# facebookresearch/momentum

Measured on AMD Instinct MI355X. Metric: character IK solves/sec (72-joint, 10 GN iters), higher is better.
Workload: dtype f32; 1 GPU; BASELINE configs[1]: B x 72-joint humanoid, P=128, pos+ori on 16 landmarks (M=192), GN lambda=0.05, 10 it; batch_per_gpu=4096, global_batch=4096, joints=72, params=128, rows=192, solved_parameters=96, route=fused, line_search=0, precision=f32

## Files before the change

momentum_amd/csrc/mmx_fused.hip:

```cpp
#include "mmx_device.hpp"
#include "mmx_fused_helpers.hpp"
#include "mmx_kernels.hpp"
#include "mmx_mixed.hpp"
#include "mmx_tree.hpp"

#include <cfloat>
#include <cstdlib>

namespace mmx {

struct MixRowRec {
  int4 q{0, 0, 0, 0};
  bool has = false;
};
template <typename Gather, typename Store>
__device__ __forceinline__ void mixTransformRows(const RigView& rig, int tid, Gather x, Store out, const MixRowRec& regRec = MixRowRec{}) {
  if (regRec.has) {
    if (tid < rig.numRowRec) {
      const int4 q = regRec.q;
      const int row = q.x & 0xffff, span = int(uint32_t(q.x) >> 16), in0 = q.y & 0xffff, cnt = int(uint32_t(q.y) >> 16);
      auto acc = __int_as_float(q.z) * x(in0);
      for (int k = q.w + 1; k < q.w + cnt; ++k) {
        acc += rig.ptValue[k] * x(rig.ptInner[k]);
      }
// ... 195 lines not shown
  }
  __syncthreads();
  for (int r = 0; r < rig.jumpRounds; ++r) {
    int next = -1;
    if (target >= 0) {
      const double* t = m.Y + kTanD * target;
#pragma unroll
      for (int c = 0; c < 7; ++c) {
        acc[c] += t[c];
      }
      next = reinterpret_cast<const int*>(t + 7)[0];
    }
    __syncthreads();
    if (target >= 0) {
      double* o = m.Y + kTanD * tid;
#pragma unroll
      for (int c = 0; c < 7; ++c) {
        o[c] = acc[c];
      }
      reinterpret_cast<int*>(o + 7)[0] = next;
    }
    target = next;
    __syncthreads();
  }
}

template <class FV>
__device__ __forceinline__ void mixApply(
    const RigView& rig, const FV& fd, const FusedLds& s, const MixLds& m, const int16_t* parentPos, int J, int NP, int n, int nsrc, double mu, const double* p, double* q, int tid, const MixRowRec& regRec = MixRowRec{}) {
  mixTangent(
      rig, fd, m, parentPos, J, tid,
      [&](int c) {
        const int cs = fd.colToSolve[c];
        return cs >= 0 ? p[cs] : 0.0;
      },
      regRec);
  mixAdjoint(
      fd, s, m, J, NP, n, nsrc, tid,
      [&](int u, int k, const D3& pu) {
        const double* pre = m.Y + kTanD * k;
        D3 v = dcross(D3{pre[3], pre[4], pre[5]}, pu);
        if (u < fd.Kp) {
          v = D3{pre[0], pre[1], pre[2]} + v + (kLn2D * pre[6]) * pu;
        }
        const double sg = m.us[u];
        return (sg * sg) * v;
      },
      q);
  for (int c = tid; c < n; c += 256) {
    q[c] += mu * p[c];
  }
  __syncthreads();
}

constexpr int kGenEv = 29;

template <int NB, bool kTR, bool kGen, int kRule>
struct FusedFour {
  static constexpr bool value = NB <= 6 && !kGen && !kTR;
};

struct FusedLayout {
  size_t uyFloats;
  size_t auxOff;
  size_t cellOff;
  size_t t9;
  size_t arenaFloats;
  size_t umomFloats;
  size_t regionFloats;
  size_t genFloats;
  size_t total;
};
__host__ __device__ inline FusedLayout fusedLayout(int NB, int J, int P, int U, int nsrc, int n, int numCells, bool cellsBehindRho, int GT, int genRows, bool separateUy = false, size_t csrFloats = 0, bool mix = false) {
  auto a4 = [](size_t x) { return (x + 3) & ~size_t(3); };
  auto h4 = [&](size_t x) { return a4((x + 1) / 2); };
  auto mx = [](size_t x, size_t y) { return x > y ? x : y; };
  const size_t T = size_t(NB) * (NB + 1) / 2, NP = 16 * size_t(NB);
  FusedLayout l;
  l.cellOff = cellsBehindRho ? 2 * NP : 0;
  const size_t aux = a4(mx(2 * NP, mx(size_t(nsrc), l.cellOff + size_t(numCells))));
  l.auxOff = separateUy ? a4(3 * size_t(U)) : 0;
  l.uyFloats = separateUy ? l.auxOff + aux : mx(a4(3 * size_t(U)), aux);
  l.t9 = a4(size_t(kTan) * J);
  l.arenaFloats = mx(size_t(kSrcCh - 1) * size_t(srcStrideFor(nsrc)), 2 * l.t9 + a4(P));
  if (mix) {
    l.arenaFloats = mx(size_t(kSrcCh - 1) * size_t(srcStrideFor(nsrc)), a4(2 * (mixXDoubles(J, nsrc) + mixYDoubles(J, P))));
  }
  l.umomFloats = mx(a4(size_t(kUmom) * U), a4(size_t(kC1) * J));
  const size_t scratch = fkBufFloats(J) + 2 * a4(size_t(kC2) * J) + l.umomFloats;
  l.regionFloats = mx(scratch, T * 256);
  const size_t rowsGp = a4(size_t(genRows));
  l.genFloats = GT > 0 ? a4(size_t(kGenEv) * GT) + 2 * a4(rowsGp) + a4(rowsGp * size_t(srcStrideFor(int(NP)))) : 0;
  const size_t meta = h4(NP + 1) + 3 * a4(nsrc) + a4(J) + 4 * h4(J) + h4(size_t(J) + 1) + 2 * h4(U) + h4(n) + h4(P);
  size_t fixed = a4(P) + a4(size_t(kJs) * J) + 2 * a4(3 * size_t(U)) + a4(U) + 2 * a4(NP) + l.uyFloats + 16 + 8;
  if (mix) {
    fixed = l.uyFloats + 40 + 8 + a4(2 * mixPersistentDoubles(J, P, U, int(NP))) + 2 * h4(J);
  }
  l.total = meta + fixed + l.genFloats + l.arenaFloats + l.regionFloats + csrFloats;
  return l;
}

__device__ __forceinline__ double generalRowsError(const ProblemDev& pb, const float* js, int b, int tid) {
  double e = 0.0;
  for (int g = tid; g < pb.G; g += 256) {
    const JointBlockDev k = jointBlockOf(pb, b, pb.genBlock[g]);
    e += double(evalJointConstraint(k, js, pb.genJoint[g], jointBlockSecondJoint(pb, k, g), size_t(b) * size_t(k.count) + size_t(g - k.first)).werr);
  }
  if (pb.wLimit > 0.f) {
    const float tWeightE = 1e+1f * pb.wLimit;
    for (int q = tid; q < pb.NE; q += 256) {
      e += double(evalEllipsoid(pb.ellipsoids[q], js, tWeightE).werr);
    }
  }
  return e;
}

__device__ __forceinline__ double generalRowsEvaluate(const ProblemDev& pb, const float* js, int b, int U, int tid, float* gEv, float* gRes) {
  double e = 0.0;
  int* evi = reinterpret_cast<int*>(gEv);
  for (int g = tid; g < pb.G; g += 256) {
    const JointBlockDev k = jointBlockOf(pb, b, pb.genBlock[g]);
    const int i = g - k.first;
    const JointEval o = evalJointConstraint(k, js, pb.genJoint[g], jointBlockSecondJoint(pb, k, g), size_t(b) * size_t(k.count) + size_t(i));
    const int row = k.rowStart + o.nrows * i - 3 * U;
    e += double(o.werr);
    for (int q = 0; q < o.nrows; ++q) {
      gRes[row + q] = o.sigma * o.f[q];
    }
    const float sg = fabsf(o.sigma) <= 1e-9f ? 0.f : o.sigma;
    float* w = gEv + kGenEv * g;
    w[0] = o.vp.x, w[1] = o.vp.y, w[2] = o.vp.z;
    w[3] = o.vn.x, w[4] = o.vn.y, w[5] = o.vn.z;
#pragma unroll
    for (int q = 0; q < 9; ++q) {
      w[6 + q] = sg * o.dp[q];
      w[15 + q] = sg * o.dn[q];
    }
    evi[kGenEv * g + 24] = pb.genTin[g];
    evi[kGenEv * g + 25] = row;
    evi[kGenEv * g + 26] = jointEvalFlags(o);
    evi[kGenEv * g + 27] = jointBlockSecondTin(pb, k, g);
  }
  const float tWeightE = 1e+1f * pb.wLimit;
  for (int q = tid; q < pb.NE; q += 256) {
    const EllipsoidDev ct = pb.ellipsoids[q];
    const int row = pb.rowsJoint - 3 * pb.NE + 3 * q - 3 * U, g = pb.G + q;
    EllipsoidEval o = evalEllipsoid(ct, js, tWeightE);
    if (!(pb.wLimit > 0.f)) {
      o.jwgt = o.werr = 0.f;
    }
    e += double(o.werr);
    gRes[row] = o.diff.x * o.jwgt, gRes[row + 1] = o.diff.y * o.jwgt, gRes[row + 2] = o.diff.z * o.jwgt;
    float* w = gEv + kGenEv * g;
    w[0] = o.position.x, w[1] = o.position.y, w[2] = o.position.z;
    w[3] = w[4] = w[5] = 0.f;
#pragma unroll
    for (int k = 0; k < 9; ++k) {
      w[6 + k] = (k == 0 || k == 4 || k == 8) ? o.jwgt : 0.f;
      w[15 + k] = 0.f;
    }
    evi[kGenEv * g + 24] = ct.tinParent;
    evi[kGenEv * g + 25] = row;
    evi[kGenEv * g + 26] = 3 | 16;
    evi[kGenEv * g + 27] = ct.tinStop;
  }
  return e;
}

struct GenSlot {
// ... 505 lines not shown
  SolveStateDev st;
  FusedParams fp;
};
static __global__ void stashFusedArgsKernel(FusedArgs a, FusedArgs* dst) {
  *dst = a;
}
template <int NB, int MODE, bool kTR, bool kGen = false, int kRule = -1, bool kArgLazy = false, bool kMix = false>
__global__ void __launch_bounds__(256, (NB <= 6 && !kGen ? (FusedFour<NB, kTR, kGen, kRule>::value && !kMix ? 4 : 3) : (NB <= 8 ? 2 : 1))) fusedSolveKernel(
    const FusedArgs* __restrict__ argsDev,
    const RigDev rigArg,
    const ProblemDev pbArg,
    FusedDev fdV,
    float* __restrict__ theta,
    SolveStateDev stV,
    FusedParams fpV,
    float* __restrict__ dbgH,
    float* __restrict__ dbgG,
    long long* __restrict__ dbgClk,
    MixSelect sel) {
  static_assert(!kMix || (!kTR && !kGen && kRule == -1 && !kArgLazy), "the mixed-precision instantiation: generic rule, reference rows");
  constexpr int T = NB * (NB + 1) / 2;
  constexpr int NP = 16 * NB;
  constexpr bool kLook = NB <= 8;
  long long clkLast = 0;
  const int dbgStop = (MODE == 2 && dbgClk != nullptr) ? int(dbgClk[31]) : 0;
#define MMX_CLK(slot)                                             \
  if (MODE == 2 && blockIdx.x == 0 && threadIdx.x == 0) {         \
    const long long now_ = clock64();                             \
    dbgClk[slot] += now_ - clkLast;                               \
    clkLast = now_;                                               \
  }                                                               \
  if (MODE == 2 && dbgStop == (slot) + 1) {                       \
    __builtin_amdgcn_endpgm();                                    \
  }
  extern __shared__ __attribute__((aligned(16))) float smem[];
  int bSel = blockIdx.x;
  if (kMix && sel.map != nullptr) {
    if (int(blockIdx.x) >= *sel.count) {
      return;
    }
    bSel = sel.map[blockIdx.x];
  }
  const int b = bSel, tid = threadIdx.x;
  const int wave = tid >> 6, lane = tid & 63;
  RigDev rigV;
  ProblemDev pbV;
  if (!kArgLazy) {
    rigV = rigArg;
    pbV = pbArg;
    selectInstanceRig(rigV, b);
    selectInstanceWeights(pbV, b);
  }
  const RigDev& rig = kArgLazy ? argsDev->rig : rigV;
  const ProblemDev& pb = kArgLazy ? argsDev->pb : pbV;
  const FusedDev& fd = kArgLazy ? argsDev->fd : fdV;
  const SolveStateDev& st = kArgLazy ? argsDev->st : stV;
  const FusedParams& fp = kArgLazy ? argsDev->fp : fpV;
  const int J = rig.J, P = rig.P, U = fd.U, n = fd.n, nsrc = fd.nsrc;
  const int JL = rig.layoutJ;
  const int kR = rig.R;

  FusedLds s;
  int16_t *lParentPos, *lSubSize, *lPosUnitStart, *lPosUnits, *lUnitJoint, *lSolveList, *lDfsJoint, *lLoadedPos, *lColToSolve;
  int *lParent, *lPtOuter = nullptr, *lPtInner = nullptr;
  float *srcGu, *cells, *arena, *lPtValue = nullptr;
  constexpr bool kFour = FusedFour<NB, kTR, kGen, kRule>::value && !kMix;
  constexpr bool kCsrLds = !kFour && !kMix;
  constexpr bool kLeanSolve = kFour;
  constexpr bool kRide = kFour && NB >= 2;
  constexpr bool kLeanOps = kFour;
  constexpr bool kLeanAcc = kFour;
  const int kNnz = fd.nnz;
  const FusedLayout lay = fusedLayout(NB, JL, P, U, nsrc, n, fd.numCells, kRule < 0, kGen ? fd.GT : 0, kGen ? fd.genRows : 0, kTR, 0, kMix);
  MixLds m{};
  m.layoutJ = JL;
  {
    float* p = smem;
    auto take = [&](size_t count) {
      float* r = p;
      p += alignUp4(count);
      return r;
    };
    auto takeS = [&](size_t count) { return reinterpret_cast<int16_t*>(take((count + 1) / 2)); };
    s.mStart = takeS(NP + 1);
    s.mTin = reinterpret_cast<int*>(take(nsrc));
    s.mInfo = reinterpret_cast<int*>(take(nsrc));
    s.mW = take(nsrc);
    lParent = reinterpret_cast<int*>(take(JL));
    lParentPos = takeS(JL);
    lSubSize = takeS(JL);
    lPosUnitStart = takeS(JL + 1);
    lPosUnits = takeS(U);
    lUnitJoint = takeS(U);
    lSolveList = takeS(n);
    lDfsJoint = takeS(JL);
    lLoadedPos = takeS(JL);
    lColToSolve = takeS(P);
    if (kCsrLds) {
      lPtOuter = reinterpret_cast<int*>(take(kR + 1));
      lPtInner = reinterpret_cast<int*>(take(kNnz));
      lPtValue = take(kNnz);
    }
    if (kMix) {
      s.th = s.js = s.up = s.us = s.ur = s.g = s.d0 = nullptr;
      m.lo = takeS(JL);
      m.hi = takeS(JL);
    } else {
      s.th = take(P);
      s.js = take(size_t(kJs) * JL);
      s.up = take(3 * size_t(U));
      s.ur = take(3 * size_t(U));
      s.us = take(U);
      s.g = take(NP);
      s.d0 = take(NP);
    }
    s.uy = take(lay.uyFloats);
    s.rho = s.uy + lay.auxOff, s.invDiag = s.rho + NP, srcGu = s.rho, cells = s.rho + lay.cellOff;
    s.red = reinterpret_cast<double*>(take(kMix ? 40 : 16));
    s.flags = reinterpret_cast<int*>(take(8));
    s.gEv = s.gRes = s.gW = s.gJ = nullptr;
    if (kGen) {
      const int rowsGp = (fd.genRows + 3) & ~3;
      s.gEv = take(size_t(kGenEv) * size_t(fd.GT));
      s.gRes = take(rowsGp);
      s.gW = take(rowsGp);
      s.gJ = take(size_t(rowsGp) * size_t(srcStrideFor(NP)));
    }
    arena = take(lay.arenaFloats);
    if (kMix) {
      m.X = reinterpret_cast<double*>(arena);
      m.Y = m.X + mixXDoubles(JL, nsrc);
    }
    s.srcT = arena;
    s.tanOwn = arena, s.jd = arena + lay.t9, s.tanPre = arena + lay.t9, s.dfull = arena + 2 * lay.t9;
    float* region = p;
    s.fkA = reinterpret_cast<double*>(take(fkBufFloats(JL)));
    s.fkB = reinterpret_cast<double*>(p);
    s.own2 = take(size_t(kC2) * JL);
    s.sub2 = take(size_t(kC2) * JL);
    s.umom = take(lay.umomFloats);
    s.own1 = region, s.sub1 = s.umom;
    s.L = region;
    if (kMix) {
      double* d = reinterpret_cast<double*>(smem + (lay.total - alignUp4(2 * mixPersistentDoubles(JL, P, U, NP))));
      m.th = d, d += P;
      m.js = d, d += size_t(kJsD) * JL;
      m.up = d, d += 3 * size_t(U);
      m.uf = d, d += 3 * size_t(U);
      m.us = d, d += U;
      m.g = d, d += NP;
      m.x = d, d += NP;
      m.r = d, d += NP;
      m.p = d, d += NP;
      m.q = d;
    }
  }

  float* thg = theta + size_t(b) * P;
  if (kMix) {
    const float* th0 = sel.thetaInit != nullptr ? sel.thetaInit + size_t(b) * P : thg;
    for (int i = tid; i < P; i += 256) {
      m.th[i] = double(th0[i]);
    }
  } else {
    for (int i = tid; i < P; i += 256) {
      s.th[i] = thg[i];
    }
  }
  for (int c = tid; c <= NP; c += 256) {
    s.mStart[c] = int16_t(fd.srcStart[c]);
  }
  for (int e = tid; e < nsrc; e += 256) {
    const ColumnSourceDev cs = fd.srcs[e];
    s.mTin[e] = cs.tin | (cs.tout << 16);
    s.mInfo[e] = cs.joint | (cs.dof << 12) | ((cs.parent + 1) << 16);
    s.mW[e] = cs.weight;
  }
  for (int i = tid; i < J; i += 256) {
    lParent[i] = rig.parent[i];
    lSubSize[i] = int16_t(fd.subSize[i]);
  }
  for (int i = tid; i <= J; i += 256) {
    lPosUnitStart[i] = int16_t(fd.posUnitStart[i]);
  }
  if (kCsrLds) {
    for (int i = tid; i <= kR; i += 256) {
      lPtOuter[i] = rig.ptOuter[i];
    }
    for (int i = tid; i < kNnz; i += 256) {
      lPtInner[i] = rig.ptInner[i];
      lPtValue[i] = rig.ptValue[i];
    }
  }
  for (int i = tid; i < U; i += 256) {
    lPosUnits[i] = int16_t(fd.posUnits[i]);
    lUnitJoint[i] = int16_t(pb.unitTin[i]);
  }
  for (int i = tid; i < n; i += 256) {
    lSolveList[i] = int16_t(fd.solveList[i]);
  }
  for (int i = tid; i < J; i += 256) {
    lDfsJoint[i] = int16_t(fd.dfsJoint[i]);
    lLoadedPos[i] = int16_t(i < fd.numLoaded ? fd.loadedPos[i] : 0);
  }
  for (int i = tid; i < P; i += 256) {
    lColToSolve[i] = -1;
  }
  if (kGen) {
    const int rowsGp = (fd.genRows + 3) & ~3;
    for (int i = tid; i < rowsGp * srcStrideFor(NP); i += 256) {
      s.gJ[i] = 0.f;
    }
    for (int i = tid; i < rowsGp; i += 256) {
      s.gRes[i] = 0.f;
      s.gW[i] = 0.f;
    }
  }
  __syncthreads();
  for (int i = tid; i < n; i += 256) {
    lColToSolve[fd.solveList[i]] = int16_t(i);
  }
  int numLoadedInst = fd.numLoaded;
  if (pb.instPosParent != nullptr || pb.instOriParent != nullptr) {
// ... 111 lines not shown
      e = waveReduceSum(e);
      if (lane == 0) {
        s.red[wave] = e;
      }
      __syncthreads();
      curError = (s.red[0] + s.red[1]) + (s.red[2] + s.red[3]);
      MMX_CLK(1)
    } else {
    blockFk<!kCsrLds>(rv, s, s.th, tid, true, MODE == 2 ? dbgClk : nullptr, &clkLast);
    MMX_CLK(1)
    {
      double e = 0.0;
      for (int u = tid; u < U; u += 256) {
        const Unit un = evalUnitFrom(pb, (!kLateUnit && u == tid) ? uin0 : loadUnitInput(pb, b, u), s.js, u);
        s.up[3 * u] = un.v.x, s.up[3 * u + 1] = un.v.y, s.up[3 * u + 2] = un.v.z;
        const float rx = un.sigma * un.f.x, ry = un.sigma * un.f.y, rz = un.sigma * un.f.z;
        s.ur[3 * u] = rx, s.ur[3 * u + 1] = ry, s.ur[3 * u + 2] = rz;
        s.uy[3 * u] = un.sigma * rx, s.uy[3 * u + 1] = un.sigma * ry, s.uy[3 * u + 2] = un.sigma * rz;
        s.us[u] = un.sigma;
        e += double(un.werr);
      }
      if (hasParamRows) {
        e += paramRowsError<true>(rig, pb, P, s.th, b, tid);
      }
      if (kGen) {
        e += generalRowsEvaluate(pb, s.js, b, U, tid, s.gEv, s.gRes);
      }
      e = waveReduceSum(e);
      if (lane == 0) {
        s.red[wave] = e;
      }
    }
    __syncthreads();
    curError = (s.red[0] + s.red[1]) + (s.red[2] + s.red[3]);
    }
    if (kGen) {
      generalRowsGather(
          s.js, s.gEv, s.gJ, srcStrideFor(NP), fd.GT, n, tid,
          [&](int e) {
            const int span = s.mTin[e], info = s.mInfo[e];
            return GenSlot{span & 0xffff, span >> 16, info & 0xfff, (info >> 12) & 7, (info >> 16) - 1, s.mW[e]};
          },
          [&](int c, int& e0, int& e1) { e0 = NP + s.mStart[c], e1 = NP + s.mStart[c + 1]; });
      __syncthreads();
    }
    MMX_CLK(2)
    if (kMix) {
      __syncthreads();
      mixAdjoint(
          fv, s, m, J, NP, n, nsrc, tid,
          [&](int u, int, const D3&) {
            const double sg = m.us[u];
            return (sg * sg) * D3{m.uf[3 * u], m.uf[3 * u + 1], m.uf[3 * u + 2]};
          },
          m.g);
      __syncthreads();
      MMX_CLK(5)
    }
    int newtonIter = 0, pdRetries = 0;
    for (;;) {
    int tidS = tid;
    if (kTR) {
      asm volatile("" : "+v"(tidS));
    }
    {
    const int tid = tidS;
    const int lane = tid & 63;
    const int wave = __builtin_amdgcn_readfirstlane(tid >> 6);
    const float mu = kTR ? 1e-20f + (trLambda - 1e-10f) : lambda;
    if (kMix) {
      ownSums<256, FusedViewS, true>(fv, s, s.umom, U, tid, m.up, m.us);
    } else {
      ownSums(fv, s, s.umom, U, tid);
    }
    __syncthreads();
    MMX_CLK(15)
    constexpr int kUnD = kFusedTreeUn;
    if (!kMix) {
      treeSum<kC1, true, kC1, kUnD>(fv, s.own1, s.sub1, J, wave, lane);
    }
    treeSum<kC2Used, true, kC2, kUnD>(fv, s.own2, s.sub2, J, wave, lane);
    __syncthreads();
    MMX_CLK(3)
    const int sst = srcStrideFor(nsrc);
    float* srcD = s.srcT;
    float* srcA = s.srcT + 7 * sst;
    float* srcG = srcGu;
    for (int e = tid; e < nsrc; e += 256) {
      ColumnSourceDev cs;
      {
        const int info = s.mInfo[e];
        cs.joint = info & 0xfff;
        cs.dof = (info >> 12) & 7;
        cs.parent = (info >> 16) - 1;
        cs.tin = s.mTin[e] & 0xffff;
      }
      float jaMix[kJs];
      if (kMix) {
        const double* ad = m.js + kJsD * cs.joint;
#pragma unroll
        for (int q = 0; q < kJs; ++q) {
          jaMix[q] = float(ad[q]);
        }
      }
      const float* a = kMix ? jaMix : s.js + kJs * cs.joint;
      const float* sb = s.sub2 + kC2 * cs.tin;
      const F3 ta{a[0], a[1], a[2]};
      const float m0 = sb[0];
      const F3 m1{sb[1], sb[2], sb[3]};
      F3 al, bv{0.f, 0.f, 0.f}, g0, ax;
      float bs = 0.f, tr;
      if (cs.dof < 3) {
        if (kMix) {
          const D3 ad = transAxisColD(m.js, cs.parent, cs.dof);
          al = F3{float(ad.x), float(ad.y), float(ad.z)};
        } else {
          al = transAxisCol(s.js, cs.parent, cs.dof);
        }
        g0 = m0 * al;
        ax = cross(m1, al);
        tr = dot(al, m1);
      } else if (cs.dof < 6) {
        const float* w = a + 8 + 3 * (cs.dof - 3);
        const F3 om{w[0], w[1], w[2]};
        al = F3{0.f, 0.f, 0.f} - cross(om, ta);
        bv = om;
        g0 = m0 * al + cross(om, m1);
        const float t2 = (sb[4] + sb[7] + sb[9]) + (sb[10] + sb[13] + sb[15]);
        const F3 Mo{
            (sb[4] + sb[10]) * om.x + (sb[5] + sb[11]) * om.y + (sb[6] + sb[12]) * om.z,
            (sb[5] + sb[11]) * om.x + (sb[7] + sb[13]) * om.y + (sb[8] + sb[14]) * om.z,
            (sb[6] + sb[12]) * om.x + (sb[8] + sb[14]) * om.y + (sb[9] + sb[15]) * om.z};
        ax = cross(m1, al) + (t2 * om - Mo);
        tr = dot(al, m1);
      } else {
        al = F3{0.f, 0.f, 0.f} - kLn2 * ta;
        bs = kLn2;
        g0 = m0 * al + kLn2 * m1;
        ax = cross(m1, al);
        tr = dot(al, m1) + kLn2 * (sb[4] + sb[7] + sb[9]);
      }
      const float w = s.mW[e];
      float* d = srcD + e;
      d[0] = w * g0.x, d[sst] = w * g0.y, d[2 * sst] = w * g0.z;
      d[3 * sst] = w * ax.x, d[4 * sst] = w * ax.y, d[5 * sst] = w * ax.z;
      d[6 * sst] = w * tr;
      float* o = srcA + e;
      o[0] = w * al.x, o[sst] = w * al.y, o[2 * sst] = w * al.z;
      o[3 * sst] = w * bv.x, o[4 * sst] = w * bv.y, o[5 * sst] = w * bv.z;
      o[6 * sst] = w * bs;
      if (!kMix) {
        srcG[e] = w * sourceGradient(cs.joint, cs.dof, cs.parent, s.js, s.sub1 + kC1 * cs.tin);
      }
    }
    __syncthreads();
    MMX_CLK(4)
    for (int c = tid; c < (kMix ? 0 : NP); c += 256) {
      float acc = srcG[c];
      const int e1 = NP + s.mStart[c + 1];
      for (int e = NP + s.mStart[c]; e < e1; ++e) {
        acc += srcG[e];
      }
      if (hasParamRows && c < n) {
        const ParamCol pc = paramRowsColumn(rig, pb, fd, s.th, nullptr, lColToSolve, P, b, c, lSolveList[c]);
        acc += pc.g;
        s.rho[c] = pc.h;
      }
      if (kGen && c < n) {
        const int gst = srcStrideFor(NP);
        for (int r = 0; r < fd.genRows; ++r) {
          acc += s.gJ[r * gst + c] * s.gRes[r];
        }
      }
      s.g[c] = acc;
      s.d0[c] = acc;
    }
    if (kMix && hasParamRows) {
      for (int c = tid; c < n; c += 256) {
        const ParamColD pc = paramRowsColumnD<false>(rig, pb, fd, m.th, nullptr, lColToSolve, P, b, c, lSolveList[c]);
        m.g[c] += pc.g;
        s.rho[c] = float(pc.h);
      }
    }
    MMX_CLK(5)
    {
      const int i = lane & 15, gq = lane >> 4;
      const int k1 = gq < 3 ? 4 + gq : 6;
      struct TileOps {
        float dI0, aI0, dJ0, aJ0, dI1, aI1, dJ1, aJ1;
        int spanC, spanR[4];
      };
      auto loadOps = [&](int I, int Jc) {
        TileOps o;
        const int ri = 16 * I + i, ci = 16 * Jc + i;
        o.dI0 = srcD[gq * sst + ri], o.aI0 = srcA[gq * sst + ri];
        o.dJ0 = srcD[gq * sst + ci], o.aJ0 = srcA[gq * sst + ci];
        o.dI1 = srcD[k1 * sst + ri], o.aI1 = srcA[k1 * sst + ri];
        o.dJ1 = srcD[k1 * sst + ci], o.aJ1 = srcA[k1 * sst + ci];
        o.spanC = s.mTin[ci];
#pragma unroll
        for (int q = 0; q < 4; ++q) {
          o.spanR[q] = s.mTin[16 * I + 4 * gq + q];
        }
        return o;
      };
      int I = 0, Jc = wave;
      auto normalise = [&]() {
        while (Jc > I) {
          Jc -= I + 1;
          ++I;
        }
      };
      normalise();
      TileOps cur = loadOps(I < NB ? I : 0, I < NB ? Jc : 0);
      for (int t = wave; t < T; t += 4) {
        const int tI = I, tJ = Jc;
        Jc += 4;
        normalise();
        const bool more = t + 4 < T;
        TileOps nxt;
        if (!kLeanOps) {
          nxt = loadOps(more ? I : tI, more ? Jc : tJ);
        }
        const float z = gq == 3 ? 0.f : 1.f;
        v4f P{0.f, 0.f, 0.f, 0.f}, Q{0.f, 0.f, 0.f, 0.f};
        P = __builtin_amdgcn_mfma_f32_16x16x4f32(cur.dI0, cur.aJ0, P, 0, 0, 0);
        Q = __builtin_amdgcn_mfma_f32_16x16x4f32(cur.aI0, cur.dJ0, Q, 0, 0, 0);
        P = __builtin_amdgcn_mfma_f32_16x16x4f32(z * cur.dI1, cur.aJ1, P, 0, 0, 0);
        Q = __builtin_amdgcn_mfma_f32_16x16x4f32(z * cur.aI1, cur.dJ1, Q, 0, 0, 0);
        const int tinC = cur.spanC & 0xffff, toutC = cur.spanC >> 16;
        float* Tc = s.L + 256 * tileIndex(tI, tJ);
#pragma unroll
        for (int q = 0; q < 4; ++q) {
          const int tinR = cur.spanR[q] & 0xffff, toutR = cur.spanR[q] >> 16;
          const bool rowDeep = tinC <= tinR && tinR < toutC;
          const bool colDeep = tinR <= tinC && tinC < toutR;
          Tc[tileAddr(4 * gq + q, i)] = rowDeep ? P[q] : (colDeep ? Q[q] : 0.f);
        }
        if (kLeanOps) {
          nxt = loadOps(more ? I : tI, more ? Jc : tJ);
        }
        cur = nxt;
      }
    }
    __syncthreads();
    MMX_CLK(12)
    if (fd.termRounds > 0) {
      float h = 0.f;
      constexpr int kRecTrip = 8;
      for (int k0 = 0; k0 < fd.termRounds; k0 += kRecTrip) {
        uint2 rec[kRecTrip];
#pragma unroll
        for (int k = 0; k < kRecTrip; ++k) {
          const uint4* rp = asGlobal(fd.gTerms) + (k0 + k) * 256 + tid;
          rec[k] = *reinterpret_cast<const uint2*>(rp);
        }
        if (MODE == 2) {
          asm volatile("s_waitcnt vmcnt(0)" ::: "memory");
          MMX_CLK(21)
        }
#pragma unroll
        for (int k = 0; k < kRecTrip; ++k) {
          const uint32_t x = rec[k].x;
          if (x & (1u << 26)) {
            const int deep = x & 0xfff, anc = (x >> 12) & 0xfff;
            float dv[7], av[7];
#pragma unroll
            for (int ch = 0; ch < 7; ++ch) {
              dv[ch] = srcD[ch * sst + deep];
              av[ch] = srcA[ch * sst + anc];
            }
            float hj = 0.f;
#pragma unroll
            for (int ch = 0; ch < 7; ++ch) {
              hj += dv[ch] * av[ch];
            }
            h = (x & (1u << 24)) ? hj : h + hj;
            if (x & (1u << 25)) {
              const uint32_t y = rec[k].y;
              if (y & (1u << 30)) {
                cells[y & 0xffff] = h;
              } else {
                s.L[y] += h;
              }
            }
          }
        }
        MMX_CLK(11)
      }
      __syncthreads();
    }
    if (fd.numComb > 0) {
      for (int i = tid; i < fd.numComb; i += 256) {
        const int dest = fd.comb[3 * i], first = fd.comb[3 * i + 1], cnt = fd.comb[3 * i + 2];
        float v = s.L[dest];
        for (int c = 0; c < cnt; ++c) {
          v += cells[first + c];
        }
        s.L[dest] = v;
      }
      __syncthreads();
    }
    if (hasParamRows) {
      for (int c = tid; c < n; c += 256) {
        s.L[256 * tileIndex(c >> 4, c >> 4) + tileAddr(c & 15, c & 15)] += s.rho[c];
      }
      if (pb.wLimit > 0.f) {
        const float tWeight = 1e+1f * pb.wLimit;
        for (int d = tid; d < fd.numPairDests; d += 256) {
          float accp = 0.f;
          const int k1 = fd.pairStart[d + 1];
          for (int k = fd.pairStart[d]; k < k1; ++k) {
            float ca = 0.f, cb = 0.f;
            if (kMix) {
              const LimitRowT<double> row = evalLimit<double>(rig, pb.limits[fd.pairLim[k]], m.th, pb.enabledMask, double(tWeight));
#pragma unroll
              for (int e = 0; e < kLimitEntries; ++e) {
                const int sc = row.idx[e] >= 0 ? lColToSolve[row.idx[e]] : -1;
                ca += sc == fd.pairCols[2 * d] ? float(row.coef[e]) : 0.f;
                cb += sc == fd.pairCols[2 * d + 1] ? float(row.coef[e]) : 0.f;
              }
            } else {
              const LimitRow row = evalLimit(rig, pb.limits[fd.pairLim[k]], s.th, pb.enabledMask, tWeight);
#pragma unroll
              for (int e = 0; e < kLimitEntries; ++e) {
                const int sc = row.idx[e] >= 0 ? lColToSolve[row.idx[e]] : -1;
                ca += sc == fd.pairCols[2 * d] ? row.coef[e] : 0.f;
                cb += sc == fd.pairCols[2 * d + 1] ? row.coef[e] : 0.f;
              }
            }
            accp += ca * cb;
          }
          s.L[fd.pairDest[d]] += accp;
        }
      }
      __syncthreads();
    }
    if (kGen) {
      const int i = lane & 15, gq = lane >> 4;
      const int gst = srcStrideFor(NP), steps = (fd.genRows + 3) >> 2;
      for (int t = wave; t < T; t += 4) {
        int I, Jc;
        tileDecode(t, I, Jc);
        v4f acc{0.f, 0.f, 0.f, 0.f};
        for (int k = 0; k < steps; ++k) {
          const float* rowp = s.gJ + (4 * k + gq) * gst;
          acc = __builtin_amdgcn_mfma_f32_16x16x4f32(rowp[16 * I + i], rowp[16 * Jc + i], acc, 0, 0, 0);
        }
        float* Tc = s.L + 256 * t;
#pragma unroll
        for (int q = 0; q < 4; ++q) {
          Tc[tileAddr(4 * gq + q, i)] += acc[q];
        }
// ... 34 lines not shown
    }
    __syncthreads();
    MMX_CLK(6)

    for (int k = 0; k < NB; ++k) {
      auto updateTile = [&](int I, int kc, int j0, int j1) {
        float* Tc = s.L + 256 * tileIndex(I, kc);
        v4f c0, c1{0.f, 0.f, 0.f, 0.f};
#pragma unroll
        for (int r = 0; r < 4; ++r) {
          c0[r] = Tc[tileAddr(4 * (lane >> 4) + r, lane & 15)];
        }
        for (int j = j0; j < j1; ++j) {
          const float4 av = ldsRow4(s.L + 256 * tileIndex(I, j), lane & 15, lane >> 4);
          const float4 bv = ldsRow4(s.L + 256 * tileIndex(kc, j), lane & 15, lane >> 4);
          if ((j & 1) && !kLeanAcc) {
            c1 = __builtin_amdgcn_mfma_f32_16x16x4f32(-av.x, bv.x, c1, 0, 0, 0);
            c1 = __builtin_amdgcn_mfma_f32_16x16x4f32(-av.y, bv.y, c1, 0, 0, 0);
            c1 = __builtin_amdgcn_mfma_f32_16x16x4f32(-av.z, bv.z, c1, 0, 0, 0);
            c1 = __builtin_amdgcn_mfma_f32_16x16x4f32(-av.w, bv.w, c1, 0, 0, 0);
          } else {
            c0 = __builtin_amdgcn_mfma_f32_16x16x4f32(-av.x, bv.x, c0, 0, 0, 0);
            c0 = __builtin_amdgcn_mfma_f32_16x16x4f32(-av.y, bv.y, c0, 0, 0, 0);
            c0 = __builtin_amdgcn_mfma_f32_16x16x4f32(-av.z, bv.z, c0, 0, 0, 0);
            c0 = __builtin_amdgcn_mfma_f32_16x16x4f32(-av.w, bv.w, c0, 0, 0, 0);
          }
        }
#pragma unroll
        for (int r = 0; r < 4; ++r) {
          Tc[tileAddr(4 * (lane >> 4) + r, lane & 15)] = c0[r] + c1[r];
        }
      };
      if (k > 0) {
        const int jFirst = (kLook && k >= 2) ? k - 1 : 0;
        for (int I = k + wave; I < NB; I += 4) {
          updateTile(I, k, jFirst, k);
        }
        __syncthreads();
      }
      MMX_CLK(14)
      {
        float* Dk = s.L + 256 * tileIndex(k, k);
        const bool diagLane = lane < 16;
        const int vrow = 48 * wave + (lane - 16);
        const bool identLane = !diagLane && vrow < 16;
        const int prow = 16 * k + vrow;
        const bool panelLane = !diagLane && !identLane && prow < NP;
        const bool waveWorks = wave == 0 || 16 * k + 48 * wave < NP;
        if (kRide && wave == 3 && k >= 1) {
          solveForwardBlockAhead<NB>(s.L, s.invDiag, s.d0, k - 1, lane);
        }
        if (kLook && !waveWorks && k >= 1 && k + 1 < NB) {
          const int firstIdle = (NP - 16 * k + 47) / 48;
          for (int I = k + 1 + (wave - firstIdle); I < NB; I += 4 - firstIdle) {
            updateTile(I, k + 1, 0, k);
          }
        }
        float* Tl = panelLane ? s.L + 256 * tileIndex(prow >> 4, k) : Dk;
        const int trow = diagLane ? lane : (panelLane ? (prow & 15) : vrow);
        float a[16];
        auto loadRows = [&]() {
#pragma unroll
          for (int q = 0; q < 4; ++q) {
            const float4 v = (diagLane || panelLane) ? ldsRow4(Tl, trow, q) : float4{0.f, 0.f, 0.f, 0.f};
            a[4 * q] = v.x, a[4 * q + 1] = v.y, a[4 * q + 2] = v.z, a[4 * q + 3] = v.w;
          }
          if (identLane) {
            int vr = vrow;
            asm volatile("" : "+v"(vr));
#pragma unroll
            for (int c = 0; c < 16; ++c) {
              a[c] = c == vr ? 1.f : 0.f;
            }
          }
        };
        if (waveWorks) {
          loadRows();
        }
        MMX_CLK(22)
        float invd = 0.f;
        bool bad = false;
        if (waveWorks) {
          auto chain = [&](const bool kGuard, const float floorRow) {
#pragma unroll
            for (int j = 0; j < 16; ++j) {
              const float djj = readLaneF(a[j], j);
              bad = bad || !(djj > 0.f);
              float inv = __builtin_amdgcn_rsqf(djj);
              if (kGuard) {
                const float fl = readLaneF(floorRow, j);
                inv = djj > fl ? inv : (kMix ? __builtin_amdgcn_rsqf(fl) : 0.f);
              }
              a[j] *= inv;
              if (lane == j) {
                invd = inv;
              }
              panelRowUpdate(a, j);
            }
          };
          chain(false, 0.f);
          const float floorRow = s.invDiag[16 * k + (lane & 15)];
          pivotWorst = floorRow * invd * invd > pivotWorst ? floorRow * invd * invd : pivotWorst;
          if (__any(diagLane && !(floorRow * invd * invd < 1.f))) {
            loadRows();
            chain(true, floorRow);
          }
        }
        __syncthreads();
        if (waveWorks) {
          MMX_CLK(23)
          const bool stores = panelLane || (diagLane && wave == 0);
          float v[16];
#pragma unroll
          for (int c = 0; c < 16; ++c) {
            const float partner = __int_as_float(__builtin_amdgcn_ds_swizzle(__float_as_int(a[c]), 0x401F));
            v[c] = (diagLane && c > lane) ? partner : a[c];
          }
          if (stores) {
#pragma unroll
            for (int q = 0; q < 4; ++q) {
              *reinterpret_cast<float4*>(Tl + trow * 16 + (((q ^ (trow >> 2)) & 3) << 2)) =
                  float4{v[4 * q], v[4 * q + 1], v[4 * q + 2], v[4 * q + 3]};
            }
          }
          if (diagLane && wave == 0) {
            s.invDiag[16 * k + lane] = invd;
            if (bad) {
              s.flags[1] = 1;
            }
          }
        }
        __syncthreads();
        for (int r = 16 * (k + 1) + 176 + tid; r < NP; r += 256) {
          float* Tr = s.L + 256 * tileIndex(r >> 4, k);
          float x[16];
#pragma unroll
          for (int q = 0; q < 4; ++q) {
            const float4 v = ldsRow4(Tr, r & 15, q);
            x[4 * q] = v.x, x[4 * q + 1] = v.y, x[4 * q + 2] = v.z, x[4 * q + 3] = v.w;
          }
#pragma unroll
          for (int j = 0; j < 16; ++j) {
            float sum = x[j];
#pragma unroll
            for (int c = 0; c < j; ++c) {
              sum -= x[c] * Dk[tileAddr(j, c)];
            }
            x[j] = sum * s.invDiag[16 * k + j];
          }
#pragma unroll
          for (int c = 0; c < 16; ++c) {
            Tr[tileAddr(r & 15, c)] = x[c];
          }
        }
        if (NP - 16 * (k + 1) > 176) {
          __syncthreads();
        }
      }
      MMX_CLK(13)
    }
    __syncthreads();
    badPivot = s.flags[1] != 0;
    MMX_CLK(7)

    if (kMix) {
      for (int c = tid; c < NP; c += 256) {
        const double gc = c < n ? m.g[c] : 0.0;
        m.x[c] = 0.0;
        m.r[c] = gc;
        s.rho[c] = float(gc);
      }
      __syncthreads();
      solveLLt<NB, false>(s.L, s.invDiag, s.rho, tid);
      double rz = 0.0;
      for (int c = tid; c < n; c += 256) {
        const double z = double(s.rho[c]);
        m.p[c] = z;
        rz += m.r[c] * z;
      }
      rz = blockSumD(s.red, rz, tid);
      MMX_CLK(16)
      const double tol2 = double(fp.mixTol) * double(fp.mixTol);
      bool converged = !(rz > 0.0);
      for (int k = 0; k < fp.mixMaxCg && !converged; ++k) {
        mixApply(rv, fv, s, m, lParentPos, J, NP, n, nsrc, double(mu), m.p, m.q, tid, mixRecP);
        if (hasParamRows) {
          for (int c = tid; c < n; c += 256) {
            m.q[c] += paramRowsColumnD<true>(rig, pb, fd, m.th, m.p, lColToSolve, P, b, c, lSolveList[c]).g;
          }
          __syncthreads();
        }
        ++mixApplied;
        MMX_CLK(17)
        double pq = 0.0;
        for (int c = tid; c < n; c += 256) {
          pq += m.p[c] * m.q[c];
        }
        pq = blockSumD(s.red, pq, tid);
        if (!(pq > 0.0)) {
// ... 1728 lines not shown
```

momentum_amd/csrc/mmx_fused_helpers.hpp:

```cpp
#pragma once

#include "mmx_device.hpp"
#include "mmx_kernels.hpp"
#include "mmx_tree.hpp"

namespace mmx {

struct FusedLds {
  int16_t* mStart;
  int* mTin;
  int* mInfo;
  float* mW;
  float* th;
  float* js;
  float* up;
  float* ur;
  float* uy;
  float* us;
  float* own1;
  float* sub1;
  float* g;
  float* d0;
  float* rho;
  float* invDiag;
  float* dfull;
  float* jd;
  float* tanOwn;
  float* tanPre;
  double* red;
  int* flags;
  float* gEv;
  float* gRes;
  float* gW;
  float* gJ;
  double* fkA;
  double* fkB;
  float* own2;
  float* umom;
  float* sub2;
  float* L;
  float* srcT;
};

struct RigView {
  int32_t J, P, R, numLevels, jumpRounds;
  const int32_t* parent;
  const float* preRot;
  const float* offset;
  const int32_t* ptOuter;
  const int32_t* ptInner;
  const float* ptValue;
  const float* ptOffsets;
  bool hasOffsets;
  const int32_t* levelOrder;
  const int32_t* levelStart;
  const int4* rowRec;
  int32_t numRowRec;
};
template <class I>
struct FusedViewT {
  int32_t U, Kp;
  const I* subSize;
  const I* dfsJoint;
  const I* loadedPos;
  int32_t numLoaded;
  const I* colToSolve;
  const I* unitPos;
  const I* posUnitStart;
  const I* posUnits;
  const I* solveList;
};
using FusedView = FusedViewT<int32_t>;
using FusedViewS = FusedViewT<int16_t>;

__host__ __device__ __forceinline__ size_t alignUp4(size_t x) {
  return (x + 3) & ~size_t(3);
}
__host__ __device__ __forceinline__ int srcStrideFor(int nsrc) {
  int x = (nsrc + 15) & ~15;
  return (x & 31) == 16 ? x : x + 16;
}
constexpr int kSrcCh = 15;

__device__ __forceinline__ void firstOrderMoments(float* o, F3 p, float yx, float yy, float yz, bool point) {
  o[3] = p.y * yz - p.z * yy;
  o[4] = p.z * yx - p.x * yz;
  o[5] = p.x * yy - p.y * yx;
  o[0] = point ? yx : 0.f;
  o[1] = point ? yy : 0.f;
  o[2] = point ? yz : 0.f;
  o[6] = point ? p.x * yx + p.y * yy + p.z * yz : 0.f;
}

template <int NCH, int STRIDE, int kT = 256, class FV = FusedView, bool kSecondOnly = false>
__device__ __forceinline__ void gatherOwnSums(const FV& fd, const FusedLds& s, const float* umom, int tid) {
  for (int item = tid; item < fd.numLoaded * NCH; item += kT) {
    const int li = item / NCH, c = item - li * NCH;
    const int k = fd.loadedPos[li];
    float acc = 0.f;
    const int e1 = fd.posUnitStart[k + 1];
    for (int e = fd.posUnitStart[k]; e < e1; ++e) {
      acc += umom[STRIDE * fd.posUnits[e] + c];
    }
    if (kSecondOnly) {
      s.own2[kC2 * k + c] = acc;
    } else if (c < kC1) {
      s.own1[kC1 * k + c] = acc;
    } else {
      s.own2[kC2 * k + (c - kC1)] = acc;
    }
  }
}
constexpr int kUmom = 25;

template <int kT = 256, class FV = FusedView, bool kSecondOnly = false>
__device__ __forceinline__ void ownSums(const FV& fd, const FusedLds& s, float* umom, int U, int tid, const double* upD = nullptr, const double* usD = nullptr) {
  constexpr int NCH = kSecondOnly ? kC2Used : kC1 + kC2Used;
  for (int u = tid; u < U; u += kT) {
    const F3 p = kSecondOnly ? F3{float(upD[3 * u]), float(upD[3 * u + 1]), float(upD[3 * u + 2])} : F3{s.up[3 * u], s.up[3 * u + 1], s.up[3 * u + 2]};
    const bool point = u < fd.Kp;
    float* o = umom + kUmom * u;
    if (!kSecondOnly) {
      firstOrderMoments(o, p, s.uy[3 * u], s.uy[3 * u + 1], s.uy[3 * u + 2], point);
    }
    const float sg = kSecondOnly ? float(usD[u]) : s.us[u];
    const float s2 = sg * sg;
    float* o2 = kSecondOnly ? o : o + kC1;
#pragma unroll
    for (int c = 0; c < kC2Used; ++c) {
      o2[c] = 0.f;
    }
    const int q = point ? 4 : 10;
    o2[q + 0] = s2 * p.x * p.x;
    o2[q + 1] = s2 * p.x * p.y;
    o2[q + 2] = s2 * p.x * p.z;
    o2[q + 3] = s2 * p.y * p.y;
    o2[q + 4] = s2 * p.y * p.z;
    o2[q + 5] = s2 * p.z * p.z;
    if (point) {
      o2[0] = s2;
      o2[1] = s2 * p.x;
      o2[2] = s2 * p.y;
      o2[3] = s2 * p.z;
    }
  }
  __syncthreads();
  gatherOwnSums<NCH, kUmom, kT, FV, kSecondOnly>(fd, s, umom, tid);
}

constexpr int kFusedTreeUn = 4;
template <int NC, bool kSubtree, int STRIDE = NC, int UN = kFusedTreeUn, class I = int32_t>
__device__ __forceinline__ void treeSum(const FusedViewT<I>& fd, const float* in, float* out, int J, int wave, int lane, const int32_t* kRange = nullptr) {
  treeSumT<NC, kSubtree, STRIDE, UN, I>(fd.subSize, fd.loadedPos, fd.numLoaded, in, out, J, wave, 4, lane, kRange);
}

struct ParamCol {
  float g, h;
};

template <class I = int32_t>
__device__ __forceinline__ ParamCol paramRowsColumn(
    const RigDev& rig,
    const ProblemDev& pb,
    const FusedDev& fd,
    const float* th,
// ... 229 lines not shown
```

Before: 2.243 million solves/s.

## Interleave per-source D/A channels into contiguous 14-float slots

Changes the source table from channel-major (stride sst per channel) to source-major interleaved slots of 14 floats, so each source's D and A channels sit contiguously. Each column's writes and the tile-ops and deep/ancestor reads now hit adjacent LDS addresses, aiming for fewer address computations and better vectorizable LDS accesses. It also forces layout sizes to be wave-uniform via readfirstlane and uses opaque lane copies to steer codegen in the Cholesky panel. Stride 14 may cause LDS bank conflicts for strided lane access, and the diagLane condition removed from the v[] select changes values for non-diagonal lanes, which relies on those lanes' outputs being unused or identical.

```diff
diff --git a/momentum_amd/csrc/mmx_fused.hip b/momentum_amd/csrc/mmx_fused.hip
--- a/momentum_amd/csrc/mmx_fused.hip
+++ b/momentum_amd/csrc/mmx_fused.hip
@@ -301,9 +301,9 @@
   l.auxOff = separateUy ? a4(3 * size_t(U)) : 0;
   l.uyFloats = separateUy ? l.auxOff + aux : mx(a4(3 * size_t(U)), aux);
   l.t9 = a4(size_t(kTan) * J);
-  l.arenaFloats = mx(size_t(kSrcCh - 1) * size_t(srcStrideFor(nsrc)), 2 * l.t9 + a4(P));
+  l.arenaFloats = mx(slotTableFloats(nsrc), 2 * l.t9 + a4(P));
   if (mix) {
-    l.arenaFloats = mx(size_t(kSrcCh - 1) * size_t(srcStrideFor(nsrc)), a4(2 * (mixXDoubles(J, nsrc) + mixYDoubles(J, P))));
+    l.arenaFloats = mx(slotTableFloats(nsrc), a4(2 * (mixXDoubles(J, nsrc) + mixYDoubles(J, P))));
   }
   l.umomFloats = mx(a4(size_t(kUmom) * U), a4(size_t(kC1) * J));
   const size_t scratch = fkBufFloats(J) + 2 * a4(size_t(kC2) * J) + l.umomFloats;
@@ -975,6 +975,7 @@
       return r;
     };
     auto takeS = [&](size_t count) { return reinterpret_cast<int16_t*>(take((count + 1) / 2)); };
+    auto uniform = [](size_t count) { return size_t(uint32_t(__builtin_amdgcn_readfirstlane(int(count)))); };
     s.mStart = takeS(NP + 1);
     s.mTin = reinterpret_cast<int*>(take(nsrc));
     s.mInfo = reinterpret_cast<int*>(take(nsrc));
@@ -1007,7 +1008,7 @@
       s.g = take(NP);
       s.d0 = take(NP);
     }
-    s.uy = take(lay.uyFloats);
+    s.uy = take(uniform(lay.uyFloats));
     s.rho = s.uy + lay.auxOff, s.invDiag = s.rho + NP, srcGu = s.rho, cells = s.rho + lay.cellOff;
     s.red = reinterpret_cast<double*>(take(kMix ? 40 : 16));
     s.flags = reinterpret_cast<int*>(take(8));
@@ -1019,7 +1020,7 @@
       s.gW = take(rowsGp);
       s.gJ = take(size_t(rowsGp) * size_t(srcStrideFor(NP)));
     }
-    arena = take(lay.arenaFloats);
+    arena = take(uniform(lay.arenaFloats));
     if (kMix) {
       m.X = reinterpret_cast<double*>(arena);
       m.Y = m.X + mixXDoubles(JL, nsrc);
@@ -1031,7 +1032,7 @@
     s.fkB = reinterpret_cast<double*>(p);
     s.own2 = take(size_t(kC2) * JL);
     s.sub2 = take(size_t(kC2) * JL);
-    s.umom = take(lay.umomFloats);
+    s.umom = take(uniform(lay.umomFloats));
     s.own1 = region, s.sub1 = s.umom;
     s.L = region;
     if (kMix) {
@@ -1309,9 +1310,8 @@
     treeSum<kC2Used, true, kC2, kUnD>(fv, s.own2, s.sub2, J, wave, lane);
     __syncthreads();
     MMX_CLK(3)
-    const int sst = srcStrideFor(nsrc);
     float* srcD = s.srcT;
-    float* srcA = s.srcT + 7 * sst;
+    float* srcA = s.srcT + 7;
     float* srcG = srcGu;
     for (int e = tid; e < nsrc; e += 256) {
       ColumnSourceDev cs;
@@ -1368,14 +1368,14 @@
         tr = dot(al, m1) + kLn2 * (sb[4] + sb[7] + sb[9]);
       }
       const float w = s.mW[e];
-      float* d = srcD + e;
-      d[0] = w * g0.x, d[sst] = w * g0.y, d[2 * sst] = w * g0.z;
-      d[3 * sst] = w * ax.x, d[4 * sst] = w * ax.y, d[5 * sst] = w * ax.z;
-      d[6 * sst] = w * tr;
-      float* o = srcA + e;
-      o[0] = w * al.x, o[sst] = w * al.y, o[2 * sst] = w * al.z;
-      o[3 * sst] = w * bv.x, o[4 * sst] = w * bv.y, o[5 * sst] = w * bv.z;
-      o[6 * sst] = w * bs;
+      float tv[kSlotStride] = {w * g0.x, w * g0.y, w * g0.z, w * ax.x, w * ax.y, w * ax.z, w * tr,
+                               w * al.x, w * al.y, w * al.z, w * bv.x, w * bv.y, w * bv.z, w * bs};
+      float* d = srcD + kSlotStride * e;
+#pragma unroll
+      for (int q = 0; q < kSlotStride; ++q) {
+        asm volatile("" : "+v"(tv[q]));
+        d[q] = tv[q];
+      }
       if (!kMix) {
         srcG[e] = w * sourceGradient(cs.joint, cs.dof, cs.parent, s.js, s.sub1 + kC1 * cs.tin);
       }
@@ -1420,10 +1420,12 @@
       auto loadOps = [&](int I, int Jc) {
         TileOps o;
         const int ri = 16 * I + i, ci = 16 * Jc + i;
-        o.dI0 = srcD[gq * sst + ri], o.aI0 = srcA[gq * sst + ri];
-        o.dJ0 = srcD[gq * sst + ci], o.aJ0 = srcA[gq * sst + ci];
-        o.dI1 = srcD[k1 * sst + ri], o.aI1 = srcA[k1 * sst + ri];
-        o.dJ1 = srcD[k1 * sst + ci], o.aJ1 = srcA[k1 * sst + ci];
+        const float* pr = srcD + kSlotStride * ri;
+        const float* pc = srcD + kSlotStride * ci;
+        o.dI0 = pr[gq], o.aI0 = pr[7 + gq];
+        o.dJ0 = pc[gq], o.aJ0 = pc[7 + gq];
+        o.dI1 = pr[k1], o.aI1 = pr[7 + k1];
+        o.dJ1 = pc[k1], o.aJ1 = pc[7 + k1];
         o.spanC = s.mTin[ci];
 #pragma unroll
         for (int q = 0; q < 4; ++q) {
@@ -1492,10 +1494,12 @@
           if (x & (1u << 26)) {
             const int deep = x & 0xfff, anc = (x >> 12) & 0xfff;
             float dv[7], av[7];
+            const float* pd = srcD + kSlotStride * deep;
+            const float* pa = srcA + kSlotStride * anc;
 #pragma unroll
             for (int ch = 0; ch < 7; ++ch) {
-              dv[ch] = srcD[ch * sst + deep];
-              av[ch] = srcA[ch * sst + anc];
+              dv[ch] = pd[ch];
+              av[ch] = pa[ch];
             }
             float hj = 0.f;
 #pragma unroll
@@ -1696,6 +1700,8 @@
         bool bad = false;
         if (waveWorks) {
           auto chain = [&](const bool kGuard, const float floorRow) {
+            int laneC = lane;
+            asm volatile("" : "+v"(laneC));
 #pragma unroll
             for (int j = 0; j < 16; ++j) {
               const float djj = readLaneF(a[j], j);
@@ -1706,7 +1712,7 @@
                 inv = djj > fl ? inv : (kMix ? __builtin_amdgcn_rsqf(fl) : 0.f);
               }
               a[j] *= inv;
-              if (lane == j) {
+              if (laneC == j) {
                 invd = inv;
               }
               panelRowUpdate(a, j);
@@ -1725,10 +1731,12 @@
           MMX_CLK(23)
           const bool stores = panelLane || (diagLane && wave == 0);
           float v[16];
+          int laneS = lane;
+          asm volatile("" : "+v"(laneS));
 #pragma unroll
           for (int c = 0; c < 16; ++c) {
             const float partner = __int_as_float(__builtin_amdgcn_ds_swizzle(__float_as_int(a[c]), 0x401F));
-            v[c] = (diagLane && c > lane) ? partner : a[c];
+            v[c] = c > laneS ? partner : a[c];
           }
           if (stores) {
 #pragma unroll
diff --git a/momentum_amd/csrc/mmx_fused_helpers.hpp b/momentum_amd/csrc/mmx_fused_helpers.hpp
--- a/momentum_amd/csrc/mmx_fused_helpers.hpp
+++ b/momentum_amd/csrc/mmx_fused_helpers.hpp
@@ -81,6 +81,10 @@
   return (x & 31) == 16 ? x : x + 16;
 }
 constexpr int kSrcCh = 15;
+constexpr int kSlotStride = 14;
+__host__ __device__ __forceinline__ size_t slotTableFloats(int nsrc) {
+  return size_t(kSlotStride) * size_t((nsrc + 15) & ~15);
+}
 
 __device__ __forceinline__ void firstOrderMoments(float* o, F3 p, float yx, float yy, float yz, bool point) {
   o[3] = p.y * yz - p.z * yy;
```

Measured after the change: 2.342 million solves/s (median of 6 runs). 1.04x the previous value.
